# frasermince/gym-cellular-automata

Measured on AMD Instinct MI355X. Metric: cell-updates/sec, 4096x(256x256) ForestFireBulldozer (Alexandridis CA), per-GPU batch, higher is better.
Workload: dtype u8 cells / i16 ages / f32 probabilities

## Files before the change

### gym-cellular-automata_amd/csrc/gca_alex_march.hip

```cpp
#include "gca_alex_rule.h"

#include <type_traits>

#ifndef GCA_MARCH_FLAT_OCC
#define GCA_MARCH_FLAT_OCC 4
#endif
#ifndef GCA_MARCH_OBS_FLAT_OCC
#define GCA_MARCH_OBS_FLAT_OCC 3
#endif
#ifndef GCA_MARCH_XROW
#define GCA_MARCH_XROW 1
#endif

namespace {

constexpr int MW = 256;
constexpr int SH = 16;

struct MarchObs {
    const float4* col;
    const int32_t* night;
    float* rgb;
    const int32_t* action;
    int action_stride, n_choices;
    uint32_t mode_bits;
    uint8_t* refit;
};
constexpr uint32_t OBS_GRID = 0u, OBS_ZERO = 1u, OBS_NONE = 2u;
constexpr uint32_t OBS_CHK_GRID = 4u, OBS_CHK_BLUR = 8u;

__device__ __forceinline__ uint32_t from_prev(uint32_t v) {
    return (uint32_t)__builtin_amdgcn_mov_dpp((int)v, 0x138, 0xF, 0xF, true);
}
__device__ __forceinline__ uint32_t from_next(uint32_t v) {
    return (uint32_t)__builtin_amdgcn_mov_dpp((int)v, 0x130, 0xF, 0xF, true);
}
__device__ __forceinline__ uint32_t from_prev_or(uint32_t old, uint32_t v) {
    return (uint32_t)__builtin_amdgcn_update_dpp((int)old, (int)v, 0x138, 0xF, 0xF, false);
}
__device__ __forceinline__ uint32_t from_next_or(uint32_t old, uint32_t v) {
    return (uint32_t)__builtin_amdgcn_update_dpp((int)old, (int)v, 0x130, 0xF, 0xF, false);
}

__host__ __device__ constexpr uint32_t win_mask(int o, int j, int k) {
    uint32_t m = 0;
    for (int b = 0; b < 4; ++b) {
        const int c = 4 * o + b - j;
        if (c >= -k && c <= k) m |= 1u << (8 * b);
    }
    return m;
}
__host__ __device__ constexpr bool win_full(int o, int j, int k) { return j - k <= 4 * o && 4 * o + 3 <= j + k; }
template <bool HALO = false>
__device__ __forceinline__ void window4(uint32_t X, int k, uint32_t (&B)[4], uint32_t z = 0u, uint32_t h1 = 0u,
                                        uint32_t h2 = 0u) {
    uint32_t n[5] = {0u, 0u, X, 0u, 0u};
    if (k >= 1) {
        n[1] = HALO ? from_prev_or(h1, X) : from_prev(X);
        n[3] = HALO ? from_next_or(h1, X) : from_next(X);
    }
    if (k >= 5) {
        n[0] = HALO ? from_prev_or(h2, n[1]) : from_prev(n[1]);
        n[4] = HALO ? from_next_or(h2, n[3]) : from_next(n[3]);
    }
    constexpr uint32_t ONES = 0x01010101u;
    bool use0 = false, useL = false, useR = false, useLR = false;
#pragma unroll
    for (int j = 0; j < 4; ++j) {
        const bool f0 = win_full(0, j, k), fl = win_full(-1, j, k), fr = win_full(1, j, k);
        if (f0 && fl && fr) useLR = true;
        else if (f0 && fl) useL = true;
        else if (f0 && fr) useR = true;
        else if (f0) use0 = true;
    }
    uint32_t S0 = 0u, SL = 0u, SR = 0u, SLR = 0u;
    if (use0 || useL || useR || useLR) S0 = __builtin_amdgcn_udot4(n[2], ONES, z, false);
    if (useL || useLR) SL = __builtin_amdgcn_udot4(n[1], ONES, S0, false);
    if (useR) SR = __builtin_amdgcn_udot4(n[3], ONES, S0, false);
    if (useLR) SLR = __builtin_amdgcn_udot4(n[3], ONES, SL, false);
#pragma unroll
    for (int j = 0; j < 4; ++j) {
        const bool f0 = win_full(0, j, k), fl = win_full(-1, j, k), fr = win_full(1, j, k);
        const bool run = f0;
        uint32_t acc = !run ? z : (fl && fr) ? SLR : fl ? SL : fr ? SR : S0;
#pragma unroll
        for (int o = -2; o <= 2; ++o) {
            if (run && (o == 0 || (o == -1 && fl) || (o == 1 && fr))) continue;
            const uint32_t m = win_mask(o, j, k);
            if (m) acc = __builtin_amdgcn_udot4(n[o + 2], m, acc, false);
        }
        B[j] = acc;
    }
}

__device__ __forceinline__ float4 ldf4(const float* p) { return *reinterpret_cast<const float4*>(p); }
__device__ __forceinline__ gca_f2 m_recip(float v0, float v1) {
    const gca_f2 x = {v0, v1};
    const gca_f2 r0 = {__builtin_amdgcn_rcpf(v0), __builtin_amdgcn_rcpf(v1)};
    const gca_f2 ee = __builtin_elementwise_fma(-x, r0, (gca_f2){1.0f, 1.0f});
    return __builtin_elementwise_fma(ee, r0, r0);
}
__device__ __forceinline__ void m_edge_both(float v0, float v1, gca_f2& own, gca_f2& nb) {
    const gca_f2 rc = m_recip(v0, v1);
    asm("v_max_f32_e64 %0, %1, -%2" : "=v"(own.x) : "v"(v0), "v"(rc.x));
    asm("v_max_f32_e64 %0, %1, -%2" : "=v"(own.y) : "v"(v1), "v"(rc.y));
    asm("v_max_f32_e64 %0, -%1, %2" : "=v"(nb.x) : "v"(v0), "v"(rc.x));
    asm("v_max_f32_e64 %0, -%1, %2" : "=v"(nb.y) : "v"(v1), "v"(rc.y));
}
__device__ __forceinline__ void m_edge_both4(const float4& v, gca_f2& oa, gca_f2& na, gca_f2& ob, gca_f2& nb) {
    const gca_f2 x0 = {v.x, v.y}, x1 = {v.z, v.w};
    const gca_f2 r0 = {__builtin_amdgcn_rcpf(v.x), __builtin_amdgcn_rcpf(v.y)};
    const gca_f2 r1 = {__builtin_amdgcn_rcpf(v.z), __builtin_amdgcn_rcpf(v.w)};
    const gca_f2 e0 = __builtin_elementwise_fma(-x0, r0, (gca_f2){1.0f, 1.0f});
    const gca_f2 e1 = __builtin_elementwise_fma(-x1, r1, (gca_f2){1.0f, 1.0f});
    const gca_f2 c0 = __builtin_elementwise_fma(e0, r0, r0);
    const gca_f2 c1 = __builtin_elementwise_fma(e1, r1, r1);
    asm("v_max_f32_e64 %0, %1, -%2" : "=v"(oa.x) : "v"(v.x), "v"(c0.x));
    asm("v_max_f32_e64 %0, %1, -%2" : "=v"(oa.y) : "v"(v.y), "v"(c0.y));
    asm("v_max_f32_e64 %0, %1, -%2" : "=v"(ob.x) : "v"(v.z), "v"(c1.x));
    asm("v_max_f32_e64 %0, %1, -%2" : "=v"(ob.y) : "v"(v.w), "v"(c1.y));
    asm("v_max_f32_e64 %0, -%1, %2" : "=v"(na.x) : "v"(v.x), "v"(c0.x));
    asm("v_max_f32_e64 %0, -%1, %2" : "=v"(na.y) : "v"(v.y), "v"(c0.y));
    asm("v_max_f32_e64 %0, -%1, %2" : "=v"(nb.x) : "v"(v.z), "v"(c1.x));
    asm("v_max_f32_e64 %0, -%1, %2" : "=v"(nb.y) : "v"(v.w), "v"(c1.y));
}
__device__ __forceinline__ void m_edge_own4(const float4& v, gca_f2& oa, gca_f2& ob) {
    const gca_f2 x0 = {v.x, v.y}, x1 = {v.z, v.w};
    const gca_f2 r0 = {__builtin_amdgcn_rcpf(v.x), __builtin_amdgcn_rcpf(v.y)};
    const gca_f2 r1 = {__builtin_amdgcn_rcpf(v.z), __builtin_amdgcn_rcpf(v.w)};
    const gca_f2 e0 = __builtin_elementwise_fma(-x0, r0, (gca_f2){1.0f, 1.0f});
    const gca_f2 e1 = __builtin_elementwise_fma(-x1, r1, (gca_f2){1.0f, 1.0f});
    const gca_f2 c0 = __builtin_elementwise_fma(e0, r0, r0);
    const gca_f2 c1 = __builtin_elementwise_fma(e1, r1, r1);
    asm("v_max_f32_e64 %0, %1, -%2" : "=v"(oa.x) : "v"(v.x), "v"(c0.x));
    asm("v_max_f32_e64 %0, %1, -%2" : "=v"(oa.y) : "v"(v.y), "v"(c0.y));
    asm("v_max_f32_e64 %0, %1, -%2" : "=v"(ob.x) : "v"(v.z), "v"(c1.x));
    asm("v_max_f32_e64 %0, %1, -%2" : "=v"(ob.y) : "v"(v.w), "v"(c1.y));
}
template <class T, class B> __device__ __forceinline__ T ld_at(const B* base, uint32_t off) {
    return *reinterpret_cast<const T*>(reinterpret_cast<const unsigned char*>(base) + off);
}
template <class T, class B> __device__ __forceinline__ T ld_nt(const B* base, uint32_t off) {
    constexpr int N = (int)(sizeof(T) / 4);
    typedef uint32_t vt __attribute__((ext_vector_type(N)));
    typedef const __attribute__((address_space(1))) unsigned char gbyte;
    typedef const __attribute__((address_space(1))) vt gvt;
    const vt v = __builtin_nontemporal_load((gvt*)((gbyte*)base + off));
    return __builtin_bit_cast(T, v);
}
constexpr uint32_t WZ = 0x4B000000u;
__device__ __forceinline__ gca_f2 wsum_f2(uint32_t b0, uint32_t b1) {
    return (gca_f2){__uint_as_float(b0), __uint_as_float(b1)} - (gca_f2){8388608.0f, 8388608.0f};
}
typedef uint16_t u16x2 __attribute__((ext_vector_type(2)));
typedef int16_t i16x2 __attribute__((ext_vector_type(2)));
__device__ __forceinline__ i16x2 bitcast_i16x2(uint32_t v) { return __builtin_bit_cast(i16x2, v); }
__device__ __forceinline__ u16x2 bitcast_u16x2(uint32_t v) { return __builtin_bit_cast(u16x2, v); }
template <class T> __device__ __forceinline__ uint32_t bitcast_u32(T v) { return __builtin_bit_cast(uint32_t, v); }

constexpr int XI = 16;
constexpr int XS_ONE = 13, XS_TWO = 14;

template <int R, bool OBS, bool GROW, int NSEG, int FLATM>
__global__ __launch_bounds__(NSEG == 1 ? 256 : 64 * NSEG) __attribute__((amdgpu_waves_per_eu(OBS ? (FLATM ? GCA_MARCH_OBS_FLAT_OCC : 2) : (FLATM ? GCA_MARCH_FLAT_OCC : 3), OBS ? (FLATM ? GCA_MARCH_OBS_FLAT_OCC : 2) : (FLATM ? GCA_MARCH_FLAT_OCC : 3)))) void alex_march_kernel(
    gca_alex_params p, int H, int nwaves, const uint8_t* __restrict__ grid_in, uint8_t* __restrict__ grid_out,
    const int16_t* age_in, int16_t* age_out,
    const uint8_t* __restrict__ vd, const uint16_t* __restrict__ dbits, const float* __restrict__ es,
    const int32_t* __restrict__ wind_index, const uint32_t* __restrict__ rng_step, int32_t* __restrict__ counts,
    const uint8_t* __restrict__ act_in, uint8_t* __restrict__ act_out, MarchObs obs) {
    constexpr int NF = 2 * R + 2;
    constexpr bool HALO = NSEG > 1;
    constexpr int WPB = HALO ? NSEG : 4;
    constexpr int W = MW * NSEG;
    __shared__ float lut[WPB][16];
    __shared__ float4 colw[WPB][8];
    __shared__ float4 img[OBS ? WPB : 1][OBS ? 192 : 1];
    __shared__ uint32_t fring[WPB][2 * NF * 64];
    __shared__ uint32_t xch[HALO ? 2 : 1][HALO ? NSEG + 2 : 1][4][HALO ? XI : 1];
    __shared__ uint32_t qfl[HALO ? NSEG : 1];
    constexpr bool FLAT = FLATM >= 1, UNI = FLATM == 2;
    constexpr bool XROW = GCA_MARCH_XROW && !HALO && OBS && !FLAT;
    __shared__ float4 xrow[XROW ? 4 : 1][3][XROW ? 64 : 1];
    __shared__ uint32_t xok[XROW ? 4 : 1];

    const int tid = threadIdx.x, wl = __builtin_amdgcn_readfirstlane(tid >> 6), lane = tid & 63;
    const int nb = (int)gridDim.x;
    const int xcd = (int)blockIdx.x & 7, slot = (int)blockIdx.x >> 3;
    const int qn8 = nb >> 3, rn8 = nb & 7;
    const int lb = (xcd < rn8 ? xcd * (qn8 + 1) : rn8 * (qn8 + 1) + (xcd - rn8) * qn8) + slot;
    int strips, e, s, g;
    if constexpr (!HALO) {
        const int wv = lb * 4 + wl;
        if (wv >= nwaves) {
            if constexpr (XROW) {
                if (lane == 0) xok[wl] = 0u;
                __builtin_amdgcn_fence(__ATOMIC_RELEASE, "workgroup", "local");
                __builtin_amdgcn_s_barrier();
            }
            return;
        }
        strips = H / SH;
        e = wv / strips;
        s = wv - e * strips;
        g = 0;
    } else {
        if (lb * NSEG >= nwaves) return;
        strips = H / SH;
        e = lb / strips;
        s = lb - e * strips;
        g = wl;
    }
    const int s0 = s * SH;
    const uint32_t HW = (uint32_t)H * W;
    const uint8_t* gE = grid_in + (size_t)e * HW;
    uint8_t* gO = grid_out + (size_t)e * HW;
    const int16_t* aE = age_in + (size_t)e * HW;
    int16_t* aO = age_out + (size_t)e * HW;
    const uint8_t* vE = UNI ? vd : vd + (size_t)e * HW;
    const uint16_t* dE = dbits + (size_t)e * (HW >> 4);
    const float* sE = FLAT ? es : es + (size_t)e * 4 * HW;
    const uint32_t lc = HALO ? (uint32_t)(MW * g) + 4u * (uint32_t)lane : 4u * (uint32_t)lane;
    const uint32_t ld16 = HALO ? lc >> 4 : (uint32_t)(lane >> 2);
    const uint32_t lane_a = 2u * lc, lane_s = 4u * lc, lane_d = 2u * ld16;
    const uint32_t Fp = rep4((uint32_t)p.fire), Ep = rep4((uint32_t)p.empty), Tp = rep4((uint32_t)p.tree);

    if (lane < 16) lut[wl][lane] = gca_alex_lut_entry(p, lane);
    if (OBS && lane < 6) colw[wl][lane] = obs.col[6 * (obs.night[e] != 0 ? 1 : 0) + lane];
    uint32_t omode = 0u;
    if constexpr (OBS && !HALO) {
        if (obs.action) {
            const int choice = min(max(obs.action[(size_t)e * obs.action_stride + 2], 0), obs.n_choices - 1);
            omode = (uint32_t)__builtin_amdgcn_readfirstlane((int)((obs.mode_bits >> (4 * choice)) & 0xFu));
        }
    }
    auto row0_refit = [&](uint32_t x0, uint32_t x1) -> uint8_t {
        const uint32_t odd = ((x0 + 0x7D7D7D7Du) | x0 | (x1 + 0x7D7D7D7Du) | x1) & 0x80808080u;
        bool pos = false;
        if (omode & OBS_CHK_GRID) pos |= __ballot(x0 != 0u) != 0ull;
        if (omode & OBS_CHK_BLUR) {
            auto hsum = [&](uint32_t x) {
                uint32_t L = __builtin_amdgcn_alignbyte(x, from_prev(x), 3);
                uint32_t Rt = __builtin_amdgcn_alignbyte(from_next(x), x, 1);
                if (lane == 0) L = (x << 8) | (x & 0xFFu);
                if (lane == 63) Rt = (x >> 8) | (x & 0xFF000000u);
                return L + x + Rt;
            };
            const uint32_t S = 2u * hsum(x0) + hsum(x1);
            pos |= __ballot(((S + 0x7B7B7B7Bu) & 0x80808080u) != 0u) != 0ull;
        }
        const bool bad = __ballot(odd != 0u) != 0ull;
        return ((omode & 3u) == OBS_NONE || bad || ((omode & (OBS_CHK_GRID | OBS_CHK_BLUR)) && !pos)) ? 1 : 0;
    };
    __builtin_amdgcn_fence(__ATOMIC_RELEASE, "wavefront");
    __builtin_amdgcn_wave_barrier();
    __builtin_amdgcn_fence(__ATOMIC_ACQUIRE, "wavefront");

    auto graw = [&](int r) -> uint32_t {
        return (r >= 0 && r < H) ? *reinterpret_cast<const uint32_t*>(gE + (uint32_t)r * W + lc) : Ep;
    };
    auto draw_bits = [&](int r) -> uint32_t {
        return (r >= 0 && r < H) ? (uint32_t)dE[(uint32_t)r * (W / 16) + ld16] : 0u;
    };
    auto dflags = [&](uint32_t w16) -> uint32_t { return gca_spread4(w16 >> (4 * (lane & 3))); };
// ... 52 lines not shown
            const uint32_t o = (uint32_t)r * W + lc;
            const uint32_t gw = row(i);
            __builtin_nontemporal_store(gw, reinterpret_cast<uint32_t*>(gO + o));
            if (age_in != age_out) *reinterpret_cast<uint2*>(aO + o) = *reinterpret_cast<const uint2*>(aE + o);
            cE += __builtin_popcount(bytes_eq01(gw, Ep));
            cT += __builtin_popcount(bytes_eq01(gw, Tp));
            if (OBS) write_rgb_row(r, gca_eq_nib(gw, Tp), 0u, dflags(draw_bits(r)));
        }
        if constexpr (OBS && !HALO) {
            if (obs.refit && s0 == 0) {
                const uint8_t rf = row0_refit(row(0), row(1));
                if (lane == 0) obs.refit[e] = rf;
            }
        }
        if (act_out && lane == 0) act_out[((size_t)e * strips + s) * NSEG + g] = 0;
        if (counts) {
#pragma unroll
            for (int off = 32; off > 0; off >>= 1) {
                cE += __shfl_xor(cE, off);
                cT += __shfl_xor(cT, off);
            }
            if (lane == 0) {
                if (cE) atomicAdd(counts + 3 * e + 0, cE);
                if (cT) atomicAdd(counts + 3 * e + 1, cT);
            }
        }
    };
    bool quiet = false;
    if (!HALO && act_out && act_in) {
        const uint8_t* A = act_in + (size_t)e * strips;
        quiet = !(A[s] | (s > 0 ? A[s - 1] : 0) | (s + 1 < strips ? A[s + 1] : 0));
    } else if constexpr (!GROW) {
        auto has_fire = [&](uint32_t x) {
            const uint32_t v = x ^ Fp;
            return (v - 0x01010101u) & ~v & 0x80808080u;
        };
        if (__ballot((has_fire(g_init[R]) | has_fire(g_init[R + 1])) != 0u) == 0ull) {
            uint32_t gq[SH];
            gq[0] = g_init[R + 1];
            uint32_t f = has_fire(graw(s0 + SH));
#pragma unroll
            for (int i = 1; i < SH; ++i) {
                gq[i] = graw(s0 + i);
                f |= has_fire(gq[i]);
            }
            quiet = __ballot(f != 0u) == 0ull;
            if constexpr (!HALO) {
                if (quiet) {
                    xrow_publish(false, nullptr);
                    quiet_copy([&](int i) { return gq[i]; });
                    return;
                }
            }
        }
    }
    if constexpr (HALO) {
        if (wl == 0) {
#pragma unroll
            for (int j = 0; j < 4; ++j) {
                const int idx = 4 * lane + j;
                const int item = idx & 15, li = (idx >> 4) & 3, sl = ((idx >> 6) & 1) ? NSEG + 1 : 0, pa = idx >> 7;
                xch[pa][sl][li][item] = (item == XS_ONE || item == XS_TWO) ? 0x3F800000u : 0u;
            }
        }
        if (lane == 0) qfl[wl] = quiet ? 1u : 0u;
        __builtin_amdgcn_fence(__ATOMIC_RELEASE, "workgroup", "local");
        __builtin_amdgcn_s_barrier();
        __builtin_amdgcn_fence(__ATOMIC_ACQUIRE, "workgroup", "local");
        uint32_t all = 1u;
#pragma unroll
        for (int w = 0; w < NSEG; ++w) all &= qfl[w];
        quiet = all != 0u;
    }
    if (quiet) {
        xrow_publish(false, nullptr);
        quiet_copy([&](int i) { return *reinterpret_cast<const uint32_t*>(gE + (uint32_t)(s0 + i) * W + lc); });
        return;
    }

    uint32_t* FR = fring[wl];
    auto ring_put = [&](int t, uint32_t v) {
        const int sl = (2 * NF - 2 - t) % NF;
        FR[sl * 64 + lane] = v;
        FR[(sl + NF) * 64 + lane] = v;
    };
#pragma unroll
    for (int t = 0; t < NF - 1; ++t) ring_put(t, bytes_eq01(g_init[t], Fp));
    uint32_t dring[6];
#pragma unroll
    for (int t = 0; t < 5; ++t) dring[t] = dflags(draw_bits(s0 - 3 + t));
    uint32_t nG = graw(s0 + R), nD = draw_bits(s0 + 2), nOwn = graw(s0);
    uint32_t nVD = UNI ? 0u : *reinterpret_cast<const uint32_t*>(vE + (size_t)s0 * W + lc);
    uint2 nAge = *reinterpret_cast<const uint2*>(aE + (size_t)s0 * W + lc);
    float4 sc[4], sn[4];
#pragma unroll
    for (int k = 0; k < 4; ++k) {
        if constexpr (FLAT) {
            sc[k] = sn[k] = make_float4(1.0f, 1.0f, 1.0f, 1.0f);
        } else {
            sc[k] = ldf4(sE + (size_t)k * HW + (size_t)s0 * W + lc);
            sn[k] = ldf4(sE + (size_t)k * HW + (size_t)min(s0 + 1, H - 1) * W + lc);
        }
    }
    __builtin_amdgcn_fence(__ATOMIC_RELEASE, "wavefront");
    __builtin_amdgcn_wave_barrier();
    __builtin_amdgcn_fence(__ATOMIC_ACQUIRE, "wavefront");
    xrow_publish(true, sc);
    const bool xuse = XROW && wl < 3 && s0 + SH < H && xok[XROW ? wl + 1 : 0] != 0u;
    uint32_t V[R + 1];
#pragma unroll
    for (int k = 1; k <= R; ++k) {
        uint32_t v = 0u;
#pragma unroll
        for (int t = R - k; t <= R + k; ++t) v += FR[((2 * NF - 2 - t) % NF) * 64 + lane];
        V[k] = v;
    }
    uint32_t Dv1 = dring[1] + dring[2] + dring[3];
    uint32_t Dv2 = dring[0] + Dv1 + dring[4];

    const bool col_lo = lane == 0 && (!HALO || g == 0), col_hi = lane == 63 && (!HALO || g == NSEG - 1);
    const uint32_t xo1 = HALO ? (lane == 63 ? (uint32_t)(((g + 2) * 4 + 0) * XI) : (uint32_t)((g * 4 + 3) * XI)) : 0u;
    const uint32_t xo2 = HALO ? (lane == 63 ? (uint32_t)(((g + 2) * 4 + 1) * XI) : (uint32_t)((g * 4 + 2) * XI)) : 0u;
    auto prep_own = [&](float4& v) {
        gca_f2 a, b;
        m_edge_own4(v, a, b);
        v = make_float4(col_lo ? 1.0f : a.x, a.y, b.x, col_hi ? 1.0f : b.y);
    };
    if constexpr (!FLAT) {
#pragma unroll
        for (int k = 0; k < 3; ++k) prep_own(sc[k]);
    }

    constexpr int NHW = (R + 2) / 2;
    gca_f2 windp[4], hdwp[NHW];
    {
        const int widx = wind_index[e];
#pragma unroll
        for (int q = 0; q < 4; ++q) {
            const int d0 = 2 * q, d1 = 2 * q + 1;
            windp[q] = (gca_f2){p.winds[widx][d0 < 4 ? d0 : d0 + 1], p.winds[widx][d1 < 4 ? d1 : d1 + 1]};
            asm volatile("" : "+v"(windp[q]));
        }
#pragma unroll
        for (int q = 0; q < NHW; ++q) {
            hdwp[q] = (gca_f2){p.heat_dw[2 * q], 2 * q + 1 <= R ? p.heat_dw[2 * q + 1] : 0.0f};
            asm volatile("" : "+v"(hdwp[q]));
        }
    }
    gca_f2 avd = {1.0f, 1.0f};
    if constexpr (UNI) {
        const int b = p.vd_uniform & 0xFF;
        avd = (gca_f2){gca_alex_lut_entry(p, b & 7), gca_alex_lut_entry(p, 8 + ((b >> 4) & 7))};
        asm volatile("" : "+v"(avd));
    }
    auto bcast = [](gca_f2 v, int h) -> gca_f2 {
        return h ? __builtin_shufflevector(v, v, 1, 1) : __builtin_shufflevector(v, v, 0, 0);
    };
    const uint32_t step = rng_step ? rng_step[e] : 0u;
    const uint32_t k0 = (uint32_t)p.seed, k1 = (uint32_t)(p.seed >> 32);
    const uint32_t env_id = (uint32_t)(p.env_offset + e);
    constexpr uint32_t PM0 = 0xD2511F53u, PM1 = 0xCD9E8D57u, PW0 = 0x9E3779B9u, PW1 = 0xBB67AE85u;
    const uint64_t pq1 = (uint64_t)PM1 * step;
    const uint32_t pu0 = (uint32_t)(pq1 >> 32) ^ env_id ^ k0;
    const uint64_t pq2 = (uint64_t)PM0 * pu0;
    const uint32_t pkc = (uint32_t)GCA_TAG_ALEX_CELL ^ k1;
    const uint32_t pkc_age = (uint32_t)GCA_TAG_ALEX_AGE ^ k1;
    const uint32_t pka = (uint32_t)pq1 ^ (k0 + PW0);
    const uint32_t pkb = (uint32_t)(pq2 >> 32) ^ (k1 + PW1);
    const uint32_t pl2 = (uint32_t)pq2;
    auto philox_cell = [&](uint32_t x0, uint32_t rk0, uint32_t rk1, uint32_t ktag) -> u32x4 {
        const uint64_t p0 = (uint64_t)PM0 * x0;
        const uint32_t hi0 = (uint32_t)(p0 >> 32), lo0 = (uint32_t)p0;
        const uint64_t p1 = (uint64_t)PM1 * (hi0 ^ ktag);
        u32x4 c = u32x4{(uint32_t)(p1 >> 32) ^ pka, (uint32_t)p1, lo0 ^ pkb, pl2};
#pragma unroll
        for (int i = 2; i < 10; ++i) {
            const uint64_t a = (uint64_t)PM0 * c.x;
            const uint64_t b = (uint64_t)PM1 * c.z;
            const uint32_t n0 = __builtin_amdgcn_bitop3_b32((uint32_t)(b >> 32), c.y, rk0 + (uint32_t)i * PW0, 0x96);
            const uint32_t n2 = __builtin_amdgcn_bitop3_b32((uint32_t)(a >> 32), c.w, rk1 + (uint32_t)i * PW1, 0x96);
            c = u32x4{n0, (uint32_t)b, n2, (uint32_t)a};
        }
        return c;
    };
    const float pt24 = __fmul_rn(p.p_tree, 16777216.0f);
    const float w_in_minus_bd = __fsub_rn(p.dous_inner, p.dous_border);
    const uint32_t codes = (p.empty & 0xFFu) | ((p.tree & 0xFFu) << 8) | ((p.fire & 0xFFu) << 16);
    int cntE = 0, cntT = 0, cntF = 0;
    uint32_t out_row0 = 0u;

    auto row = [&](const int i, float4 (&SC)[4], float4 (&SN)[4], auto parity) {
        const int r = s0 + i;
        const uint32_t gnew = nG, dnew = nD, own = nOwn, vdw = nVD;
        const uint2 agep = nAge;
        {
            const int rg = r + 1 + R, rd = r + 3;
            const uint32_t r1 = (uint32_t)min(r + 1, H - 1);
            const uint32_t gl = ld_at<uint32_t>(gE + (size_t)min(rg, H - 1) * W, lc);
            const uint32_t d = ld_at<uint16_t>(dE + (size_t)min(rd, H - 1) * (W / 16), lane_d);
            nOwn = ld_at<uint32_t>(gE + (size_t)r1 * W, lc);
            if constexpr (!UNI) nVD = ld_nt<uint32_t>(vE + (size_t)r1 * W, lc);
            nAge = ld_nt<uint2>(aE + (size_t)r1 * W, lane_a);
            nG = rg < H ? gl : Ep;
            nD = rd < H ? d : 0u;
        }
        bool need_next = i + 1 < SH;
        auto load_next_slopes = [&]() {
            if constexpr (XROW) {
                if (i == SH - 2 && xuse) {
#pragma unroll
                    for (int k = 0; k < 3; ++k) SC[k] = xrow[wl + 1][k][lane];
                    SC[3] = SC[2];
                    return;
                }
            }
            const bool need3 = need_next && i + 2 < SH;
            const float* sb = need_next ? sE : es;
            const float* sb3 = need3 ? sE : es;
            const uint32_t rs = need_next ? (uint32_t)min(r + 2, H - 1) : 0u;
            const uint32_t rs3 = need3 ? rs : 0u;
#pragma unroll
            for (int k = 0; k < 4; ++k)
                SC[k] = ld_nt<float4>((k == 3 ? sb3 : sb) + (size_t)k * HW + (size_t)(k == 3 ? rs3 : rs) * W, lane_s);
        };
        uint32_t* Fb = FR + (NF - 1 - (uint32_t)i % NF) * 64;
        {
            const uint32_t fnew = bytes_eq01(gnew, Fp);
            Fb[lane] = fnew;
            Fb[NF * 64 + lane] = fnew;
        }
        __builtin_amdgcn_fence(__ATOMIC_RELEASE, "wavefront");
        __builtin_amdgcn_wave_barrier();
        __builtin_amdgcn_fence(__ATOMIC_ACQUIRE, "wavefront");
        uint32_t fm1, f0, fp1;
        {
            uint32_t rw[NF];
#pragma unroll
            for (int t = 0; t < NF; ++t) rw[t] = Fb[(NF - 1 - t) * 64 + lane];
#pragma unroll
            for (int k = 1; k <= R; ++k) V[k] += rw[R + 1 + k] - rw[R - k];
            fm1 = rw[R];
            f0 = rw[R + 1];
            fp1 = rw[R + 2];
            if constexpr (R >= 3)
                need_next = need_next && __ballot((rw[R + 1] | rw[R + 2] | rw[R + 3] | rw[R + 4]) != 0u) != 0ull;
        }
        dring[5] = dflags(dnew);
        Dv1 += dring[4] - dring[1];
        Dv2 += dring[5] - dring[0];

        const uint32_t* xr = nullptr;
        const uint32_t* xr2 = nullptr;
        uint32_t hfm1 = 0u, hf0 = 0u, hfp1 = 0u;
        if constexpr (HALO) {
            constexpr int PAR = decltype(parity)::value;
            if (lane < 2 || lane >= 62) {
                const int xl = lane < 2 ? lane : lane - 60;
                uint4* xd = reinterpret_cast<uint4*>(&xch[PAR][g + 1][xl][0]);
                uint32_t vv[8];
#pragma unroll
                for (int k = 0; k < 8; ++k) vv[k] = k + 1 <= R ? V[k + 1] : 0u;
                const uint32_t sA = lane < 32 ? __float_as_uint(SC[3].x) : __float_as_uint(SN[2].w);
                xd[0] = make_uint4(vv[0], vv[1], vv[2], vv[3]);
                xd[1] = make_uint4(vv[4], vv[5], vv[6], vv[7]);
                xd[2] = make_uint4(Dv1, Dv2, fm1, f0);
                xd[3] = make_uint4(fp1, sA, __float_as_uint(SN[0].x), 0u);
            }
            __builtin_amdgcn_fence(__ATOMIC_RELEASE, "workgroup", "local");
            __builtin_amdgcn_s_barrier();
            __builtin_amdgcn_fence(__ATOMIC_ACQUIRE, "workgroup", "local");
            xr = &xch[PAR][0][0][0] + xo1;
            xr2 = &xch[PAR][0][0][0] + xo2;
            hfm1 = xr[10];
            hf0 = xr[11];
            hfp1 = xr[12];
        }

        const uint32_t treeB = gca_eq_nib(own, Tp), emptyB = gca_eq_nib(own, Ep);
        auto shl_c = [](uint32_t x, uint32_t h) {
            return __builtin_amdgcn_alignbyte(x, HALO ? from_prev_or(h, x) : from_prev(x), 3);
        };
        auto shr_c = [](uint32_t x, uint32_t h) {
            return __builtin_amdgcn_alignbyte(HALO ? from_next_or(h, x) : from_next(x), x, 1);
        };
        auto dir_mask = [&](int d) -> uint32_t {
            const uint32_t row = d < 3 ? fm1 : (d < 5 ? f0 : fp1);
            const uint32_t hrow = d < 3 ? hfm1 : (d < 5 ? hf0 : hfp1);
            const int dc = d < 3 ? d - 1 : (d == 3 ? -1 : (d == 4 ? 1 : d - 6));
            uint32_t m = dc < 0 ? shl_c(row, hrow) : (dc > 0 ? shr_c(row, hrow) : row);
            m *= 0xFFu;
            asm volatile("" : "+v"(m));
            return m;
        };
        const uint32_t fireB = (f0 * 0x01020408u) >> 24;
        const uint32_t vor = fm1 | f0 | fp1, hvor = hfm1 | hf0 | hfp1;
        const uint32_t anyfire = (((vor | shl_c(vor, hvor) | shr_c(vor, hvor)) & 0x01010101u) * 0x01020408u) >> 24;
        gca_f2 qn[2] = {{1.0f, 1.0f}, {1.0f, 1.0f}};
        const bool row_need = __ballot((treeB & anyfire) != 0u) != 0ull;
        const bool kill_row = r == 0 || r == H - 1;
        const bool kill_next = r + 1 == H - 1;
        auto prep_next = [&](int k, bool want_nb, float (&nbv)[4]) {
            gca_f2 oa, ob, na, nb2;
            if (want_nb) {
                m_edge_both4(SN[k], oa, na, ob, nb2);
                nbv[0] = na.x; nbv[1] = na.y; nbv[2] = nb2.x; nbv[3] = nb2.y;
            } else {
                m_edge_own4(SN[k], oa, ob);
            }
            SN[k] = make_float4(col_lo ? 1.0f : oa.x, oa.y, ob.x, col_hi ? 1.0f : ob.y);
        };
        if (!row_need) {
            if constexpr (!FLAT) {
                load_next_slopes();
                float unused[4];
#pragma unroll
                for (int k = 0; k < 3; ++k) prep_next(k, false, unused);
            }
        } else {
            gca_f2 ph[2] = {{p.heat0, p.heat0}, {p.heat0, p.heat0}};
#pragma unroll
            for (int k = 0; k <= R; ++k) {
                uint32_t B[4];
                if (k == 0) {
#pragma unroll
                    for (int j = 0; j < 4; ++j) B[j] = (f0 >> (8 * j)) & 0xFFu;
                } else {
                    if constexpr (HALO)
                        window4<true>(V[k], k, B, WZ, xr[k - 1], k >= 5 ? xr2[k - 1] : 0u);
                    else
                        window4(V[k], k, B, WZ);
                }
                gca_f2 bs[2];
#pragma unroll
                for (int h = 0; h < 2; ++h)
                    bs[h] = k == 0 ? (gca_f2){(float)B[2 * h], (float)B[2 * h + 1]} : wsum_f2(B[2 * h], B[2 * h + 1]);
#pragma unroll
                for (int h = 0; h < 2; ++h) ph[h] = __builtin_elementwise_fma(bcast(hdwp[k >> 1], k & 1), bs[h], ph[h]);
                asm volatile("" : "+v"(ph[0]), "+v"(ph[1]));
                __builtin_amdgcn_sched_barrier(0);
            }
            const bool dous_any = __ballot((Dv2 | (HALO ? xr[8] | xr[9] : 0u)) != 0u) != 0ull;
            if (dous_any) {
                uint32_t D1[4], D2[4];
                if constexpr (HALO) {
                    window4<true>(Dv1, 1, D1, WZ, xr[8]);
                    window4<true>(Dv2, 2, D2, WZ, xr[9]);
                } else {
                    window4(Dv1, 1, D1, WZ);
                    window4(Dv2, 2, D2, WZ);
                }
                gca_f2 d1[2], d2[2], dz[2];
#pragma unroll
                for (int h = 0; h < 2; ++h) d1[h] = wsum_f2(D1[2 * h], D1[2 * h + 1]);
#pragma unroll
                for (int h = 0; h < 2; ++h) d2[h] = wsum_f2(D2[2 * h], D2[2 * h + 1]);
#pragma unroll
                for (int h = 0; h < 2; ++h) dz[h] = (gca_f2){w_in_minus_bd, w_in_minus_bd} * d1[h];
#pragma unroll
                for (int h = 0; h < 2; ++h)
                    dz[h] = __builtin_elementwise_fma((gca_f2){p.dous_border, p.dous_border}, d2[h], dz[h]);
#pragma unroll
                for (int h = 0; h < 2; ++h) ph[h] = ph[h] - dz[h];
            }
            if constexpr (UNI) {
#pragma unroll
                for (int h = 0; h < 2; ++h) ph[h] = ph[h] * bcast(avd, 0);
#pragma unroll
                for (int h = 0; h < 2; ++h) ph[h] = ph[h] * bcast(avd, 1);
            } else {
                gca_f2 av[2], ad[2];
#pragma unroll
                for (int h = 0; h < 2; ++h) {
                    const uint32_t b0 = (vdw >> (16 * h)) & 0xFFu, b1 = (vdw >> (16 * h + 8)) & 0xFFu;
                    av[h] = (gca_f2){lut[wl][b0 & 7u], lut[wl][b1 & 7u]};
                    ad[h] = (gca_f2){lut[wl][8 + (b0 >> 4)], lut[wl][8 + (b1 >> 4)]};
                }
#pragma unroll
                for (int h = 0; h < 2; ++h) ph[h] = ph[h] * av[h];
#pragma unroll
                for (int h = 0; h < 2; ++h) ph[h] = ph[h] * ad[h];
            }
            auto dir_pass = [&](auto kill_tag) {
                constexpr bool KILL = decltype(kill_tag)::value;
                auto apply = [&](int d, const float (&a)[4]) {
                    asm volatile("" : "+v"(ph[0]), "+v"(ph[1]), "+v"(qn[0]), "+v"(qn[1]));
                    const gca_f2 wd2 = bcast(windp[d >> 1], d & 1);
                    const uint32_t Md = dir_mask(d);
                    gca_f2 c[2];
                    if constexpr (KILL) {
#pragma unroll
                        for (int h = 0; h < 2; ++h) c[h] = gca_pk_mul_clamp01(ph[h], wd2);
                    } else {
                        gca_f2 t[2];
#pragma unroll
                        for (int h = 0; h < 2; ++h) t[h] = ph[h] * wd2;
#pragma unroll
                        for (int h = 0; h < 2; ++h) c[h] = gca_pk_mul_clamp01(t[h], (gca_f2){a[2 * h], a[2 * h + 1]});
                    }
                    uint32_t cm[2][2];
#pragma unroll
                    for (int h = 0; h < 2; ++h) {
                        cm[h][0] = __float_as_uint(c[h].x) & (uint32_t)(int32_t)(int8_t)(Md >> (16 * h));
                        cm[h][1] = __float_as_uint(c[h].y) & (uint32_t)(int32_t)(int8_t)(Md >> (16 * h + 8));
                    }
#pragma unroll
                    for (int h = 0; h < 2; ++h)
                        qn[h] = __builtin_elementwise_fma(-qn[h], (gca_f2){__uint_as_float(cm[h][0]), __uint_as_float(cm[h][1])},
                                                          qn[h]);
                    __builtin_amdgcn_sched_barrier(0);
                };
                const float one[4] = {1.0f, 1.0f, 1.0f, 1.0f};
                uint32_t h45 = 0x3F800000u, h7 = 0x3F800000u;
                if constexpr (HALO && !KILL) {
                    gca_f2 o_, n_;
                    m_edge_both(__uint_as_float(xr[XS_ONE]), __uint_as_float(xr[XS_TWO]), o_, n_);
                    h45 = __float_as_uint(n_.x);
                    h7 = __float_as_uint(n_.y);
                }
#pragma unroll
                for (int d = 0; d < 3; ++d) {
                    const float a[4] = {SC[d].x, SC[d].y, SC[d].z, SC[d].w};
                    apply(d, KILL ? one : a);
                }
                if (KILL) {
                    apply(3, one);
                    apply(4, one);
                } else {
                    gca_f2 oa, ob, na, nb2;
                    m_edge_both4(SC[3], oa, na, ob, nb2);
                    const float a3[4] = {col_lo ? 1.0f : oa.x, oa.y, ob.x, col_hi ? 1.0f : ob.y};
                    apply(3, a3);
                    const float nx = __uint_as_float((uint32_t)__builtin_amdgcn_update_dpp(
                        (int)h45, (int)__float_as_uint(na.x), 0x130, 0xF, 0xF, false));
                    const float a4[4] = {col_lo ? 1.0f : na.y, nb2.x, nb2.y, nx};
                    apply(4, a4);
                }
                if constexpr (!FLAT) load_next_slopes();
                float nb[4];
                if constexpr (!FLAT) prep_next(2, !KILL, nb);
                if (KILL) {
                    apply(5, one);
                } else {
                    const float pv = __uint_as_float((uint32_t)__builtin_amdgcn_update_dpp(
                        (int)h45, (int)__float_as_uint(nb[3]), 0x138, 0xF, 0xF, false));
                    const float a5[4] = {pv, nb[0], nb[1], col_hi ? 1.0f : nb[2]};
                    apply(5, a5);
                }
                if constexpr (!FLAT) prep_next(1, !KILL, nb);
                if (KILL) {
                    apply(6, one);
                } else {
                    const float a6[4] = {col_lo ? 1.0f : nb[0], nb[1], nb[2], col_hi ? 1.0f : nb[3]};
                    apply(6, a6);
                }
                if constexpr (!FLAT) prep_next(0, !KILL, nb);
                if (KILL) {
                    apply(7, one);
                } else {
                    const float nx = __uint_as_float((uint32_t)__builtin_amdgcn_update_dpp(
                        (int)h7, (int)__float_as_uint(nb[0]), 0x130, 0xF, 0xF, false));
                    const float a7[4] = {col_lo ? 1.0f : nb[1], nb[2], nb[3], nx};
                    apply(7, a7);
                }
            };
            if (FLAT || kill_row)
                dir_pass(std::true_type{});
            else
                dir_pass(std::false_type{});
        }
        if (kill_next) {
#pragma unroll
            for (int k = 0; k < 3; ++k) SN[k] = make_float4(1.0f, 1.0f, 1.0f, 1.0f);
        }

        const uint32_t needB = (treeB & anyfire) | (GROW ? emptyB : 0u);
        const uint32_t lin0 = (uint32_t)r * W + lc;
        uint32_t burn = 0u, grow = 0u, NA[2];
        const bool wave_draws = __ballot(needB != 0u) != 0ull;
        uint32_t rk0 = k0, rk1 = k1;
        asm volatile("" : "+s"(rk0), "+s"(rk1));
        u32x4 X = u32x4{0u, 0u, 0u, 0u};
        if (wave_draws) X = philox_cell(lin0 >> 2, rk0, rk1, pkc);
        const uint32_t xw[4] = {X.x, X.y, X.z, X.w};
#pragma unroll
        for (int h = 0; h < 2; ++h) {
            const gca_f2 thr = __builtin_elementwise_fma(qn[h], (gca_f2){-16777216.0f, -16777216.0f},
                                                         (gca_f2){16777216.0f, 16777216.0f});
            const float u0 = (float)(xw[2 * h] >> 8), u1 = (float)(xw[2 * h + 1] >> 8);
            burn |= (u0 < thr.x ? 1u : 0u) << (2 * h);
            burn |= (u1 < thr.y ? 1u : 0u) << (2 * h + 1);
            if constexpr (GROW) {
                grow |= (u0 < pt24 ? 1u : 0u) << (2 * h);
                grow |= (u1 < pt24 ? 1u : 0u) << (2 * h + 1);
            }
        }
        burn &= treeB;
        grow &= emptyB;
        {
            const uint32_t spare = __builtin_amdgcn_perm(__builtin_amdgcn_perm(X.w, X.z, 0x0c0c0400u),
                                                         __builtin_amdgcn_perm(X.y, X.x, 0x0c0c0400u), 0x05040100u);
            const uint32_t n0 = (uint32_t)randint_ms(spare, p.age_lo, p.age_hi);
            NA[0] = NA[1] = __builtin_amdgcn_perm(n0, n0, 0x05040100u);
            if (__ballot((burn & (burn - 1u)) != 0u) != 0ull) {
                const u32x4 Y = philox_cell(lin0 >> 2, rk0, rk1, pkc_age);
                const uint32_t nk[4] = {n0, (uint32_t)randint_ms(Y.x, p.age_lo, p.age_hi),
                                        (uint32_t)randint_ms(Y.y, p.age_lo, p.age_hi),
                                        (uint32_t)randint_ms(Y.z, p.age_lo, p.age_hi)};
                uint32_t a[4];
#pragma unroll
                for (int j = 0; j < 4; ++j) {
                    const uint32_t rank = (uint32_t)__builtin_popcount(burn & ((1u << j) - 1u));
                    a[j] = rank == 0 ? nk[0] : (rank == 1 ? nk[1] : (rank == 2 ? nk[2] : nk[3]));
                }
                NA[0] = __builtin_amdgcn_perm(a[1], a[0], 0x05040100u);
                NA[1] = __builtin_amdgcn_perm(a[3], a[2], 0x05040100u);
            }
        }

        const uint32_t agw[2] = {agep.x, agep.y};
        uint32_t le1;
        if (!p.burnout_eq1) {
            const uint32_t y0 = bitcast_u32(__builtin_elementwise_sub_sat(bitcast_i16x2(agw[0]), (i16x2){2, 2}));
            const uint32_t y1 = bitcast_u32(__builtin_elementwise_sub_sat(bitcast_i16x2(agw[1]), (i16x2){2, 2}));
            le1 = ((y0 >> 15) & 1u) | ((y0 >> 30) & 2u) | ((y1 >> 13) & 4u) | ((y1 >> 28) & 8u);
        } else {
            le1 = 0u;
#pragma unroll
            for (int j = 0; j < 4; ++j)
                le1 |= ((int32_t)(int16_t)(agw[j >> 1] >> (16 * (j & 1))) == 1) ? (1u << j) : 0u;
        }
        const uint32_t newF = burn | (fireB & ~le1);
        const uint32_t newT = (treeB & ~burn) | grow;
        const uint32_t newE = (emptyB & ~grow) | (fireB & le1);
        const uint32_t keepB = ~(treeB | emptyB | fireB) & 0xFu;
        uint32_t sel = gca_spread4(newT) + 2u * gca_spread4(newF);
        sel |= (gca_spread4(keepB) * 0xFFu) & 0x07060504u;
        const uint32_t outw = __builtin_amdgcn_perm(own, codes, sel);
        uint32_t nag[2];
#pragma unroll
        for (int h = 0; h < 2; ++h) {
            const uint32_t fh = ((fireB >> (2 * h)) & 1u) | (((fireB >> (2 * h + 1)) & 1u) << 16);
            const uint32_t a1 = bitcast_u32(bitcast_u16x2(agw[h]) - bitcast_u16x2(fh));
            const uint32_t bm = (((burn >> (2 * h)) & 1u) * 0xFFFFu) | (((burn >> (2 * h + 1)) & 1u) * 0xFFFF0000u);
            nag[h] = gca_bfi32(bm, NA[h], a1);
        }
        const size_t o = (size_t)r * W + lc;
        __builtin_nontemporal_store(outw, reinterpret_cast<uint32_t*>(gO + o));
        { typedef uint32_t u2v __attribute__((ext_vector_type(2)));
          __builtin_nontemporal_store((u2v){nag[0], nag[1]}, reinterpret_cast<u2v*>(aO + o)); }
        write_rgb_row(r, newT, newF, dring[3]);
        if constexpr (OBS && !HALO) {
            if (obs.refit && r < 2) {
                if (r == 0) {
                    out_row0 = outw;
                } else {
                    const uint8_t rf = row0_refit(out_row0, outw);
                    if (lane == 0) obs.refit[e] = rf;
                }
            }
        }
        cntT += __builtin_popcount(newT);
        cntF += __builtin_popcount(newF);
        cntE += __builtin_popcount(newE);

#pragma unroll
        for (int t = 0; t < 5; ++t) dring[t] = dring[t + 1];
    };
#pragma unroll 1
    for (int i = 0; i < SH; i += 2) {
        row(i, sc, sn, std::integral_constant<int, 0>{});
        row(i + 1, sn, sc, std::integral_constant<int, 1>{});
    }

    if (counts || act_out) {
        const bool anyF = __ballot(cntF != 0) != 0ull;
        if (act_out && lane == 0) act_out[((size_t)e * strips + s) * NSEG + g] = anyF ? 1 : 0;
        if (counts) {
#pragma unroll
            for (int off = 32; off > 0; off >>= 1) {
                cntT += __shfl_xor(cntT, off);
                cntF += __shfl_xor(cntF, off);
                cntE += __shfl_xor(cntE, off);
            }
            if (lane == 0) {
                if (cntE) atomicAdd(counts + 3 * e + 0, cntE);
                if (cntT) atomicAdd(counts + 3 * e + 1, cntT);
                if (cntF) atomicAdd(counts + 3 * e + 2, cntF);
            }
        }
    }
}

template <int R, bool OBS, bool GROW, int NSEG, int FLATM>
void launch_march_n(const gca_alex_params& p, int E, int H, const uint8_t* gi, uint8_t* go, const int16_t* ai,
                    int16_t* ao, const uint8_t* vd, const uint16_t* db, const float* es, const int32_t* wi,
                    const uint32_t* rs, int32_t* counts, const uint8_t* act_in, uint8_t* act_out, MarchObs obs,
                    hipStream_t st) {
    const int nwaves = E * (H / SH) * NSEG;
    if constexpr (NSEG == 1)
        hipLaunchKernelGGL((alex_march_kernel<R, OBS, GROW, 1, FLATM>), dim3((unsigned)((nwaves + 3) / 4)), dim3(256), 0, st, p,
                           H, nwaves, gi, go, ai, ao, vd, db, es, wi, rs, counts, act_in, act_out, obs);
    else
        hipLaunchKernelGGL((alex_march_kernel<R, OBS, GROW, NSEG, FLATM>), dim3((unsigned)(nwaves / NSEG)), dim3(64 * NSEG), 0,
                           st, p, H, nwaves, gi, go, ai, ao, vd, db, es, wi, rs, counts, act_in, act_out, obs);
}
template <int R, bool OBS, bool GROW, int FLATM>
void launch_march_g(const gca_alex_params& p, int E, int H, int W, const uint8_t* gi, uint8_t* go, const int16_t* ai,
                    int16_t* ao, const uint8_t* vd, const uint16_t* db, const float* es, const int32_t* wi,
                    const uint32_t* rs, int32_t* counts, const uint8_t* act_in, uint8_t* act_out, MarchObs obs,
                    hipStream_t st) {
    if (W == MW)
        launch_march_n<R, OBS, GROW, 1, FLATM>(p, E, H, gi, go, ai, ao, vd, db, es, wi, rs, counts, act_in, act_out, obs, st);
    else if (W == 2 * MW)
        launch_march_n<R, OBS, GROW, 2, FLATM>(p, E, H, gi, go, ai, ao, vd, db, es, wi, rs, counts, act_in, act_out, obs, st);
    else
        launch_march_n<R, OBS, GROW, 4, FLATM>(p, E, H, gi, go, ai, ao, vd, db, es, wi, rs, counts, act_in, act_out, obs, st);
}
template <int R, bool OBS>
void launch_march(const gca_alex_params& p, int E, int H, int W, const uint8_t* gi, uint8_t* go, const int16_t* ai,
                  int16_t* ao, const uint8_t* vd, const uint16_t* db, const float* es, const int32_t* wi,
                  const uint32_t* rs, int32_t* counts, const uint8_t* act_in, uint8_t* act_out, MarchObs obs,
                  hipStream_t st) {
    const bool grow = p.p_tree > 0.0f;
    const int fm = es ? 0 : (vd ? 1 : 2);
#define GCA_MARCH_FM(FM)                                                                                                \
    if (grow)                                                                                                         \
        launch_march_g<R, OBS, true, FM>(p, E, H, W, gi, go, ai, ao, vd, db, es, wi, rs, counts, act_in, act_out, obs, st); \
    else                                                                                                              \
        launch_march_g<R, OBS, false, FM>(p, E, H, W, gi, go, ai, ao, vd, db, es, wi, rs, counts, act_in, act_out, obs, st);
    if (fm == 0) {
        GCA_MARCH_FM(0)
    } else if (fm == 1) {
        GCA_MARCH_FM(1)
    } else {
        GCA_MARCH_FM(2)
    }
#undef GCA_MARCH_FM
}

template <bool OBS>
void dispatch_march(const gca_alex_params& p, int E, int H, int W, const uint8_t* gi, uint8_t* go, const int16_t* ai,
                    int16_t* ao, const uint8_t* vd, const uint16_t* db, const float* es, const int32_t* wi,
                    const uint32_t* rs, int32_t* counts, const uint8_t* act_in, uint8_t* act_out, MarchObs obs,
                    hipStream_t st) {
#define GCA_MARCH_CASE(RV) \
    case RV: launch_march<RV, OBS>(p, E, H, W, gi, go, ai, ao, vd, db, es, wi, rs, counts, act_in, act_out, obs, st); break;
    switch (p.R) {
#ifdef GCA_MARCH_ANALYSIS_R6
        GCA_MARCH_CASE(6)
// ... 117 lines not shown
```

Baseline: 1230 billion.

## Add LDS neighbor ring with inline-asm direction pass and packed dozer-flag window

For the flat, non-observation, non-halo march variant, this adds a per-wave LDS ring holding -inf/0 masks for the fire neighbours of three rows. The 8-direction burn pass becomes hand-scheduled inline assembly that combines ds_read2 and packed FMA with clamp, replacing the per-direction DPP and shuffle logic. It also recomputes the vertical fire sums as nested sums instead of a running add/subtract, which shrinks the duplicated fire ring by one slot. Dozer flags are now tracked as a packed nibble history instead of a shifted register array. Together these aim to cut VALU and register work in the hot row loop, at the cost of extra LDS traffic, a wave barrier per row, and fragile hand-written assembly.

```diff
diff --git a/gym-cellular-automata_amd/csrc/gca_alex_march.hip b/gym-cellular-automata_amd/csrc/gca_alex_march.hip
--- a/gym-cellular-automata_amd/csrc/gca_alex_march.hip
+++ b/gym-cellular-automata_amd/csrc/gca_alex_march.hip
@@ -10,6 +10,15 @@
 #endif
 #ifndef GCA_MARCH_XROW
 #define GCA_MARCH_XROW 1
+#endif
+#ifndef GCA_MARCH_ARING
+#define GCA_MARCH_ARING 1
+#endif
+#ifndef GCA_MARCH_VNEST
+#define GCA_MARCH_VNEST 1
+#endif
+#ifndef GCA_MARCH_DSKIP
+#define GCA_MARCH_DSKIP 1
 #endif
 
 namespace {
@@ -175,10 +184,16 @@
     __shared__ float lut[WPB][16];
     __shared__ float4 colw[WPB][8];
     __shared__ float4 img[OBS ? WPB : 1][OBS ? 192 : 1];
-    __shared__ uint32_t fring[WPB][2 * NF * 64];
+    constexpr bool FLAT = FLATM >= 1, UNI = FLATM == 2;
+    constexpr int AROW = 258;
+    constexpr bool ARING = GCA_MARCH_ARING && FLAT && !HALO && !OBS &&
+                           16 * ((2 * NF - 1) * 64 + 3 * AROW) + 896 <= 40960;
+    constexpr bool VNEST = GCA_MARCH_VNEST && FLAT, DSKIP = GCA_MARCH_DSKIP && FLAT && !HALO && !OBS;
+    constexpr int FSLOTS = ARING ? 2 * NF - 1 : 2 * NF;
+    __shared__ uint32_t fring[WPB][FSLOTS * 64];
+    __shared__ uint32_t aring[ARING ? WPB : 1][ARING ? 3 * AROW : 1];
     __shared__ uint32_t xch[HALO ? 2 : 1][HALO ? NSEG + 2 : 1][4][HALO ? XI : 1];
     __shared__ uint32_t qfl[HALO ? NSEG : 1];
-    constexpr bool FLAT = FLATM >= 1, UNI = FLATM == 2;
     constexpr bool XROW = GCA_MARCH_XROW && !HALO && OBS && !FLAT;
     __shared__ float4 xrow[XROW ? 4 : 1][3][XROW ? 64 : 1];
     __shared__ uint32_t xok[XROW ? 4 : 1];
@@ -397,13 +412,35 @@
     auto ring_put = [&](int t, uint32_t v) {
         const int sl = (2 * NF - 2 - t) % NF;
         FR[sl * 64 + lane] = v;
-        FR[(sl + NF) * 64 + lane] = v;
+        if (sl + NF < FSLOTS) FR[(sl + NF) * 64 + lane] = v;
     };
 #pragma unroll
     for (int t = 0; t < NF - 1; ++t) ring_put(t, bytes_eq01(g_init[t], Fp));
+    constexpr uint32_t NINF = 0xFF800000u;
+    constexpr int AP3 = 1, AP0 = 65, AP1 = 130, AP2 = 194;
+    uint32_t* AL = aring[ARING ? wl : 0] + (ARING ? lane : 0);
+    auto aring_put = [&](uint32_t* A, uint32_t fl) {
+        const uint32_t m = (fl ^ 0x01010101u) * 0xFFu;
+        const uint32_t n = m & 0x80808080u;
+        A[AP0] = __builtin_amdgcn_perm(m, n, 0x04000c0cu);
+        A[AP1] = __builtin_amdgcn_perm(m, n, 0x05010c0cu);
+        A[AP2] = __builtin_amdgcn_perm(m, n, 0x06020c0cu);
+        A[AP3] = __builtin_amdgcn_perm(m, n, 0x07030c0cu);
+    };
+    if constexpr (ARING) {
+        if (lane < 6) aring[wl][(lane >> 1) * AROW + (lane & 1) * 129] = NINF;
+        aring_put(AL + 2 * AROW, bytes_eq01(g_init[R], Fp));
+        aring_put(AL, bytes_eq01(g_init[R + 1], Fp));
+    }
     uint32_t dring[6];
 #pragma unroll
     for (int t = 0; t < 5; ++t) dring[t] = dflags(draw_bits(s0 - 3 + t));
+    auto dnib = [&](uint32_t w16) -> uint32_t { return (w16 >> (4 * (lane & 3))) & 0xFu; };
+    uint32_t dpk = 0u;
+    if constexpr (DSKIP) {
+#pragma unroll
+        for (int t = 0; t < 5; ++t) dpk = (dpk << 4) | dnib(draw_bits(s0 - 3 + t));
+    }
     uint32_t nG = graw(s0 + R), nD = draw_bits(s0 + 2), nOwn = graw(s0);
     uint32_t nVD = UNI ? 0u : *reinterpret_cast<const uint32_t*>(vE + (size_t)s0 * W + lc);
     uint2 nAge = *reinterpret_cast<const uint2*>(aE + (size_t)s0 * W + lc);
@@ -422,13 +459,15 @@
     __builtin_amdgcn_fence(__ATOMIC_ACQUIRE, "wavefront");
     xrow_publish(true, sc);
     const bool xuse = XROW && wl < 3 && s0 + SH < H && xok[XROW ? wl + 1 : 0] != 0u;
-    uint32_t V[R + 1];
-#pragma unroll
-    for (int k = 1; k <= R; ++k) {
-        uint32_t v = 0u;
-#pragma unroll
-        for (int t = R - k; t <= R + k; ++t) v += FR[((2 * NF - 2 - t) % NF) * 64 + lane];
-        V[k] = v;
+    uint32_t V[R + 1] = {};
+    if constexpr (!VNEST) {
+#pragma unroll
+        for (int k = 1; k <= R; ++k) {
+            uint32_t v = 0u;
+#pragma unroll
+            for (int t = R - k; t <= R + k; ++t) v += FR[((2 * NF - 2 - t) % NF) * 64 + lane];
+            V[k] = v;
+        }
     }
     uint32_t Dv1 = dring[1] + dring[2] + dring[3];
     uint32_t Dv2 = dring[0] + Dv1 + dring[4];
@@ -504,6 +543,7 @@
     int cntE = 0, cntT = 0, cntF = 0;
     uint32_t out_row0 = 0u;
 
+    uint32_t fpos = 0u;
     auto row = [&](const int i, float4 (&SC)[4], float4 (&SN)[4], auto parity) {
         const int r = s0 + i;
         const uint32_t gnew = nG, dnew = nD, own = nOwn, vdw = nVD;
@@ -538,11 +578,16 @@
             for (int k = 0; k < 4; ++k)
                 SC[k] = ld_nt<float4>((k == 3 ? sb3 : sb) + (size_t)k * HW + (size_t)(k == 3 ? rs3 : rs) * W, lane_s);
         };
-        uint32_t* Fb = FR + (NF - 1 - (uint32_t)i % NF) * 64;
+        uint32_t im = (uint32_t)i % NF;
+        if constexpr (FLAT) {
+            im = fpos;
+            fpos = fpos + 1u == (uint32_t)NF ? 0u : fpos + 1u;
+        }
+        uint32_t* Fb = FR + (NF - 1 - im) * 64;
         {
             const uint32_t fnew = bytes_eq01(gnew, Fp);
             Fb[lane] = fnew;
-            Fb[NF * 64 + lane] = fnew;
+            if (!ARING || im != 0u) Fb[NF * 64 + lane] = fnew;
         }
         __builtin_amdgcn_fence(__ATOMIC_RELEASE, "wavefront");
         __builtin_amdgcn_wave_barrier();
@@ -553,16 +598,30 @@
 #pragma unroll
             for (int t = 0; t < NF; ++t) rw[t] = Fb[(NF - 1 - t) * 64 + lane];
 #pragma unroll
-            for (int k = 1; k <= R; ++k) V[k] += rw[R + 1 + k] - rw[R - k];
+            for (int k = 1; k <= R; ++k) {
+                if constexpr (VNEST)
+                    V[k] = (k == 1 ? rw[R + 1] : V[k - 1]) + rw[R + 1 + k] + rw[R + 1 - k];
+                else
+                    V[k] += rw[R + 1 + k] - rw[R - k];
+            }
             fm1 = rw[R];
             f0 = rw[R + 1];
             fp1 = rw[R + 2];
             if constexpr (R >= 3)
                 need_next = need_next && __ballot((rw[R + 1] | rw[R + 2] | rw[R + 3] | rw[R + 4]) != 0u) != 0ull;
         }
-        dring[5] = dflags(dnew);
-        Dv1 += dring[4] - dring[1];
-        Dv2 += dring[5] - dring[0];
+        const uint32_t i3 = (uint32_t)i % 3u;
+        const uint32_t* const Am1 = AL + (i3 == 0u ? 2u : i3 - 1u) * AROW;
+        const uint32_t* const A0 = AL + i3 * AROW;
+        uint32_t* const Ap1 = AL + (i3 == 2u ? 0u : i3 + 1u) * AROW;
+        if constexpr (ARING) aring_put(Ap1, fp1);
+        if constexpr (DSKIP) {
+            dpk = (dpk << 4) | dnib(dnew);
+        } else {
+            dring[5] = dflags(dnew);
+            Dv1 += dring[4] - dring[1];
+            Dv2 += dring[5] - dring[0];
+        }
 
         const uint32_t* xr = nullptr;
         const uint32_t* xr2 = nullptr;
@@ -654,15 +713,21 @@
                 asm volatile("" : "+v"(ph[0]), "+v"(ph[1]));
                 __builtin_amdgcn_sched_barrier(0);
             }
-            const bool dous_any = __ballot((Dv2 | (HALO ? xr[8] | xr[9] : 0u)) != 0u) != 0ull;
+            const bool dous_any = DSKIP ? __ballot((dpk & 0xFFFFFu) != 0u) != 0ull
+                                        : __ballot((Dv2 | (HALO ? xr[8] | xr[9] : 0u)) != 0u) != 0ull;
             if (dous_any) {
                 uint32_t D1[4], D2[4];
+                uint32_t s1 = Dv1, s2 = Dv2;
+                if constexpr (DSKIP) {
+                    s1 = gca_spread4(dpk >> 4) + gca_spread4(dpk >> 8) + gca_spread4(dpk >> 12);
+                    s2 = s1 + gca_spread4(dpk) + gca_spread4(dpk >> 16);
+                }
                 if constexpr (HALO) {
-                    window4<true>(Dv1, 1, D1, WZ, xr[8]);
-                    window4<true>(Dv2, 2, D2, WZ, xr[9]);
+                    window4<true>(s1, 1, D1, WZ, xr[8]);
+                    window4<true>(s2, 2, D2, WZ, xr[9]);
                 } else {
-                    window4(Dv1, 1, D1, WZ);
-                    window4(Dv2, 2, D2, WZ);
+                    window4(s1, 1, D1, WZ);
+                    window4(s2, 2, D2, WZ);
                 }
                 gca_f2 d1[2], d2[2], dz[2];
 #pragma unroll
@@ -697,6 +762,45 @@
             }
             auto dir_pass = [&](auto kill_tag) {
                 constexpr bool KILL = decltype(kill_tag)::value;
+                if constexpr (ARING && KILL) {
+                    static_assert(AP3 == 1 && AP0 == 65 && AP1 == 130 && AP2 == 194, "offsets below");
+                    typedef __attribute__((address_space(3))) const uint32_t lds_u32;
+                    const uint32_t am1 = (uint32_t)(uintptr_t)(lds_u32*)Am1, a0 = (uint32_t)(uintptr_t)(lds_u32*)A0,
+                                   ap1 = (uint32_t)(uintptr_t)(lds_u32*)Ap1;
+                    gca_f2 t0, t1, t2, t3, t4, t5, t6, t7, tx;
+#define GCA_RD2(T, B, O0, O1) "ds_read2_b32 " T ", " B " offset0:" #O0 " offset1:" #O1 "\n\t"
+#define GCA_DC_LO(C, P, W, A) "v_pk_fma_f32 " C ", " P ", " W ", " A " op_sel:[0,0,0] op_sel_hi:[1,0,1] clamp\n\t"
+#define GCA_DC_HI(C, P, W, A) "v_pk_fma_f32 " C ", " P ", " W ", " A " op_sel:[0,1,0] op_sel_hi:[1,1,1] clamp\n\t"
+#define GCA_DQ(Q, C) "v_pk_fma_f32 " Q ", " Q ", " C ", " Q " neg_lo:[1,0,0] neg_hi:[1,0,0]\n\t"
+#define GCA_DIR(H, C0, A0, C1, A1, W) \
+    GCA_DC_##H(C0, "%11", W, A0) GCA_DC_##H(C1, "%12", W, A1) "s_nop 0\n\t" GCA_DQ("%9", C0) GCA_DQ("%10", C1)
+                    asm volatile(
+                        GCA_RD2("%0", "%17", 0, 65) GCA_RD2("%1", "%17", 130, 194) GCA_RD2("%2", "%17", 65, 130)
+                        GCA_RD2("%3", "%17", 194, 1) GCA_RD2("%4", "%17", 1, 66)
+                        GCA_RD2("%5", "%18", 0, 65) GCA_RD2("%6", "%18", 130, 194) GCA_RD2("%7", "%18", 1, 66)
+                        "s_waitcnt lgkmcnt(6)\n\t" GCA_DIR(LO, "%0", "%0", "%8", "%1", "%13")
+                        "s_waitcnt lgkmcnt(4)\n\t" GCA_DIR(HI, "%2", "%2", "%3", "%3", "%13")
+                        "s_waitcnt lgkmcnt(3)\n\t" GCA_DIR(LO, "%1", "%1", "%4", "%4", "%14")
+                        GCA_RD2("%0", "%19", 0, 65) GCA_RD2("%1", "%19", 130, 194) GCA_RD2("%2", "%19", 65, 130)
+                        GCA_RD2("%3", "%19", 194, 1) GCA_RD2("%4", "%19", 1, 66)
+                        "s_waitcnt lgkmcnt(6)\n\t" GCA_DIR(HI, "%5", "%5", "%8", "%6", "%14")
+                        "s_waitcnt lgkmcnt(5)\n\t" GCA_DIR(LO, "%6", "%6", "%7", "%7", "%15")
+                        "s_waitcnt lgkmcnt(3)\n\t" GCA_DIR(HI, "%0", "%0", "%8", "%1", "%15")
+                        "s_waitcnt lgkmcnt(1)\n\t" GCA_DIR(LO, "%2", "%2", "%3", "%3", "%16")
+                        "s_waitcnt lgkmcnt(0)\n\t" GCA_DIR(HI, "%1", "%1", "%4", "%4", "%16")
+                        "s_nop 1"
+                        : "=&v"(t0), "=&v"(t1), "=&v"(t2), "=&v"(t3), "=&v"(t4), "=&v"(t5), "=&v"(t6), "=&v"(t7),
+                          "=&v"(tx), "+v"(qn[0]), "+v"(qn[1])
+                        : "v"(ph[0]), "v"(ph[1]), "v"(windp[0]), "v"(windp[1]), "v"(windp[2]), "v"(windp[3]), "v"(am1),
+                          "v"(a0), "v"(ap1)
+                        : "memory");
+#undef GCA_DIR
+#undef GCA_DQ
+#undef GCA_DC_HI
+#undef GCA_DC_LO
+#undef GCA_RD2
+                    return;
+                }
                 auto apply = [&](int d, const float (&a)[4]) {
                     asm volatile("" : "+v"(ph[0]), "+v"(ph[1]), "+v"(qn[0]), "+v"(qn[1]));
                     const gca_f2 wd2 = bcast(windp[d >> 1], d & 1);
@@ -778,6 +882,11 @@
                     apply(7, a7);
                 }
             };
+            if constexpr (ARING) {
+                __builtin_amdgcn_fence(__ATOMIC_RELEASE, "wavefront");
+                __builtin_amdgcn_wave_barrier();
+                __builtin_amdgcn_fence(__ATOMIC_ACQUIRE, "wavefront");
+            }
             if (FLAT || kill_row)
                 dir_pass(std::true_type{});
             else
@@ -878,8 +987,10 @@
         cntF += __builtin_popcount(newF);
         cntE += __builtin_popcount(newE);
 
-#pragma unroll
-        for (int t = 0; t < 5; ++t) dring[t] = dring[t + 1];
+        if constexpr (!DSKIP) {
+#pragma unroll
+            for (int t = 0; t < 5; ++t) dring[t] = dring[t + 1];
+        }
     };
 #pragma unroll 1
     for (int i = 0; i < SH; i += 2) {
```

After: 1239 billion (median of 6 runs). Within noise of the previous version (+0.7%).
